# KUIS-AI-Tekalp-Research-Group/video-compression

Hardware: AMD Instinct MI355X
Metric: frames/sec + bpp/PSNR on UVG 1080p GOP-8, 1/2/4/8 MI355X (higher is better)
Workload: dtype f32; 1 GPU; LHBDC 1080p GOP-8 inference, single lambda: 7 B-frames per GOP via Model.forward, 4 independent GOP(s) per GPU per step, hierarchy levels batched across them; gop=8, resolution=1920x1080, precision=fp32, parallelism=gop-shard x1, launch=hip-graph per GOP pass

## Files before the change

video-compression_amd/csrc/conv_split.h:

```cpp
#pragma once
#include "conv_dma.h"

typedef short bf16x8 __attribute__((ext_vector_type(8)));

template <int K> struct SplitUnits {
    static constexpr int TPU = 4;
    static constexpr int Q = (K / 2) * (K / 2);
    static constexpr int V = (K + 3) / 4;
    static constexpr int H = (K - 1 + 3) / 4;
    static constexpr int U = Q + V + H;
    static constexpr int type(int u) { return u < Q ? 0 : (u < Q + V ? 1 : 2); }
    static constexpr int ky0(int u) { return u < Q ? 2 * (u / (K / 2)) : (u < Q + V ? 4 * (u - Q) : K - 1); }
    static constexpr int kx0(int u) { return u < Q ? 2 * (u % (K / 2)) : (u < Q + V ? K - 1 : 4 * (u - Q - V)); }
    static constexpr int nvalid(int u)
    {
        return u < Q ? 4 : (u < Q + V ? (K - 4 * (u - Q) < 4 ? K - 4 * (u - Q) : 4) : (K - 1 - 4 * (u - Q - V) < 4 ? K - 1 - 4 * (u - Q - V) : 4));
    }
    static constexpr int ky(int u, int q)
    {
        const int qq = q < nvalid(u) ? q : nvalid(u) - 1;
        return type(u) == 0 ? ky0(u) + (qq >> 1) : (type(u) == 1 ? ky0(u) + qq : ky0(u));
    }
    static constexpr int kx(int u, int q)
    {
// ... 158 lines not shown
#pragma unroll
        for (int nn = 0; nn < NG; ++nn) {
            const int n = n0 + nn;
            const int co = cur.nblk * C::BN + 16 * n + 4 * q;
            unsigned char *rec = sc + ((2 * nn + (q >> 1)) * 16 + px) * 48 + 8 * (q & 1);
            f32x4 v = acc[t][n];
            f32x4 r = {0.f, 0.f, 0.f, 0.f};
            if (p.res_sp3) {
                r = vc_load_split4(rec - 8 * (q & 1), q & 1);
            } else if (p.res) {
                if (pix_ok) r = *reinterpret_cast<const f32x4 *>(p.res + (long long)cur.img * p.res_sn + (long long)oy * p.res_sh + (long long)ox * p.res_sw + co);
            }
            if (p.res_first) v += r;
#pragma unroll
            for (int e = 0; e < 4; ++e) v[e] = v[e] >= 0.0f ? v[e] : v[e] * neg;
            if (p.chscale) v *= *reinterpret_cast<const f32x4 *>(p.chscale + co);
            if (p.res && !p.res_first) v += r;
            unsigned h[4], mm[4], l[4];
#pragma unroll
            for (int e = 0; e < 4; ++e) vc_split3(v[e], h[e], mm[e], l[e]);
            const u32x2 ph = {(h[0] >> 16) | h[1], (h[2] >> 16) | h[3]};
            const u32x2 pm = {(mm[0] >> 16) | mm[1], (mm[2] >> 16) | mm[3]};
            const u32x2 pl = {(l[0] >> 16) | (l[1] & 0xffff0000u), (l[2] >> 16) | (l[3] & 0xffff0000u)};
            if constexpr (C::KO & 256) {
                VC_DMA_KEEP(ph); VC_DMA_KEEP(pm); VC_DMA_KEEP(pl);
            } else {
                *reinterpret_cast<u32x2 *>(rec) = ph;
                *reinterpret_cast<u32x2 *>(rec + 16) = pm;
                *reinterpret_cast<u32x2 *>(rec + 32) = pl;
            }
        }
        if constexpr (C::KO & 256) continue;
        asm volatile("s_waitcnt lgkmcnt(0)" ::: "memory");
        const int plane0 = (cur.nblk * C::BN + 16 * n0) >> 3;
#pragma unroll
        for (int j = 0; j < NJ; ++j) {
            const bool ok = (64 * j + lane < UNITS) && row_ok && (oxb + u_w16[j] / 3 < p.Wo);
            if (ok) {
                const vc_u32x4 val = *reinterpret_cast<const vc_u32x4 *>(sc + u_plane[j] * 768 + u_w16[j] * 16);
                if constexpr (C::KO & 128) VC_DMA_KEEP(val);
                else *reinterpret_cast<vc_u32x4 *>(outb + ((((long long)(plane0 + u_plane[j])) * p.Ho + oy) * p.Wo + oxb) * 48 + u_w16[j] * 16) = val;
            }
        }
        asm volatile("s_waitcnt lgkmcnt(0)" ::: "memory");
    }
}

template <class C, int T0 = 0, int T1 = C::WM, int SC_NG = 0>
__device__ __forceinline__ void split_epilogue(const ConvArgs &p, f32x4 (&acc)[C::WM][C::WN], const DmaTile &cur, int wave, int px, int q,
                                               unsigned char *sc = nullptr)
{
    constexpr int WM = C::WM, WN = C::WN;
    if constexpr (SC_NG > 0 || (C::A_BYTES / 8 >= 3072 && WN % 2 == 0)) {
        if (sc && p.out_sp3 && p.out_mode == VC_OUT_PLAIN) {
            constexpr int NG = SC_NG > 0 ? SC_NG : ((C::A_BYTES / 8 >= WN * 1536) ? WN : 2);
            split_epilogue_records<C, NG, T0, T1>(p, acc, cur, wave, px, q, sc);
            return;
        }
    }
    const float neg = (p.act == VC_ACT_NONE) ? 1.0f : (p.act == VC_ACT_RELU ? 0.0f : p.slope);
#pragma unroll
    for (int t = T0; t < T1; ++t) {
        const int m = WM * wave + t;
        const int oy = cur.oy0 + (m >> 1), ox = cur.ox0 + 16 * (m & 1) + px;
        const bool pix_ok = oy < p.Ho && ox < p.Wo;
#pragma unroll
        for (int n = 0; n < WN; ++n) {
            const int co = cur.nblk * C::BN + 16 * n + 4 * q;
            const bool ok = pix_ok && co < p.Cout;
            f32x4 v = acc[t][n];
            f32x4 r = {0.f, 0.f, 0.f, 0.f};
            const bool ps = p.out_mode != VC_OUT_PLAIN;
            const int cps = p.Cout >> 2;
            const int pos = ps ? co / cps : 0;
            const int cch = ps ? co - pos * cps : co;
            const int yy = ps ? 2 * oy + (pos >> 1) : oy, xx = ps ? 2 * ox + (pos & 1) : ox;
            const int oh = ps ? 2 * p.Ho : p.Ho, ow = ps ? 2 * p.Wo : p.Wo;
            if (p.res_sp3) {
                if (ok) r = vc_load_split4(reinterpret_cast<const unsigned char *>(p.res) + (long long)cur.img * p.res_sn +
                                               ((((long long)(cch >> 3)) * oh + yy) * ow + xx) * 48, (cch >> 2) & 1);
            } else if (p.res) {
                const long long r_off = (long long)cur.img * p.res_sn + (long long)yy * p.res_sh + (long long)xx * p.res_sw + cch;
                if (ok) r = *reinterpret_cast<const f32x4 *>(p.res + r_off);
            }
            if (p.res_first) v += r;
#pragma unroll
            for (int e = 0; e < 4; ++e) v[e] = v[e] >= 0.0f ? v[e] : v[e] * neg;
            if (p.chscale) v *= *reinterpret_cast<const f32x4 *>(p.chscale + min(co, p.Cout - 4));
            if (p.res && !p.res_first) v += r;
            if (p.out_sp3) {
                unsigned char *o8 = reinterpret_cast<unsigned char *>(p.out) + (long long)cur.img * p.out_sn + ((((long long)(cch >> 3)) * oh + yy) * ow + xx) * 48;
                if (ok) vc_store_split4(o8, (cch >> 2) & 1, v);
            } else {
                const long long o_off = (long long)cur.img * p.out_sn + (long long)yy * p.out_sh + (long long)xx * p.out_sw + cch;
                if (ok) *reinterpret_cast<f32x4 *>(p.out + o_off) = v;
            }
        }
    }
}

template <class C> __global__ void __launch_bounds__(512, 2) conv_split_kernel(const ConvArgs p)
{
    typedef typename C::UN UN;
    constexpr int U = C::U, WM = C::WM, WN = C::WN, NA = C::NA, RING = C::RING, D = C::D, CPL = C::CPL;
    extern __shared__ __attribute__((aligned(16))) unsigned char lds8[];

    const int tid = threadIdx.x;
    const int lane = tid & 63;
    const int wave = __builtin_amdgcn_readfirstlane(tid >> 6);
    const int grp = wave >> 2;
    const int px = lane & 15, q = lane >> 4;

    const int per_img = p.tiles_x * p.tiles_y;
    const int total = per_img * p.N * p.nblks;
    const int xcd = blockIdx.x & 7, xl = blockIdx.x >> 3;
    const int tq = total >> 3, tr = total & 7;
    const int x_start = xcd * tq + min(xcd, tr), x_count = tq + (xcd < tr ? 1 : 0);
    auto tile_at = [&](int it) {
        DmaTile t;
        const int k = it * 32 + xl;
        t.valid = k < x_count;
        const int idx = x_start + (t.valid ? k : 0);
        t.nblk = idx % p.nblks;
        const int t1 = idx / p.nblks;
        t.img = t1 / per_img;
        int tx, ty;
        vc_tile_xy(t1 - t.img * per_img, p.tiles_x, p.tiles_y, p.tile_band, tx, ty);
        t.oy0 = ty * C::TH;
        t.ox0 = tx * C::TW;
        return t;
    };
    DmaTile cur = tile_at(0);
    if (!cur.valid) return;

    const int nchunk = p.Cin / (8 * CPL);
    const int upt = nchunk * U;
    const unsigned char *const in_b = reinterpret_cast<const unsigned char *>(p.in);
    const unsigned char *const wpk = reinterpret_cast<const unsigned char *>(p.wpk);
    const long long plane = (long long)p.H * p.W * C::PXB;
    const unsigned char *const zero_lane = g_vc_dma_zero + 16 * lane;

    int a_off[NA], a_rc[NA];
#pragma unroll
    for (int k = 0; k < NA; ++k) {
        const int s = k * 512 + tid;
        const int pl = s / C::PLANE_SLOTS, s2 = s - pl * C::PLANE_SLOTS;
        const int pix = s2 / 3, piece = s2 - 3 * pix;
        const int row = pix / C::COLS, col = pix - row * C::COLS;
        a_off[k] = pl * (int)plane + (row * p.W + col) * C::PXB + piece * 16;
        a_rc[k] = (pl < CPL && s2 < 3 * C::PIX) ? (row | (col << 8)) : 0x7f7f7f;
    }
    auto tile_base = [&](const DmaTile &t) {
        return in_b + (long long)t.img * p.in_sn + ((long long)(t.oy0 - C::PAD) * p.W + (t.ox0 - C::PAD)) * C::PXB;
    };
    auto issue_a = [&](const DmaTile &t, const unsigned char *tbase, int c, int k, int buf) {
        int rc = a_rc[k], off = a_off[k];
        asm volatile("" : "+v"(rc), "+v"(off));
        const unsigned iy = (unsigned)(t.oy0 - C::PAD + (rc & 0xff)), ix = (unsigned)(t.ox0 - C::PAD + (rc >> 8));
        const bool ok = t.valid && iy < (unsigned)p.H && ix < (unsigned)p.W;
        const unsigned char *sp = ok ? tbase + ((long long)c * CPL * plane + off) : zero_lane;
        if constexpr (!(C::KO & 16)) vc_glds16<true>(sp, (unsigned)(buf * C::A_BYTES + k * 8192 + wave * 1024));
    };
    const unsigned lane16 = 16 * lane;
    unsigned gbase = 0;
    auto issue_b = [&](int g, int nblk_cur, int nblk_next) {
        const int gg = g >= upt ? g - upt : g;
        const int nblk = g >= upt ? nblk_next : nblk_cur;
        const unsigned char *sbase = wpk + ((long long)nblk * upt + gg) * (C::FRAGS * 1024) + wave * 1024;
        const unsigned dst = C::B_OFF + ((gbase + (unsigned)g) % RING) * C::SLOTB + wave * 1024;
#pragma unroll
        for (int r = 0; r < C::ROUNDS; ++r)
            if constexpr (!(C::KO & 16)) {
                if (r + 1 < C::ROUNDS || !C::EXACT || grp == 0) vc_glds16_sbase(sbase + r * 8192, lane16, dst + r * 8192);
            }
    };

    float *const ldsf = reinterpret_cast<float *>(lds8);
    for (int i = tid; i < p.nblks * C::BN; i += 512) ldsf[C::BIAS_OFF / 4 + i] = p.bias[i];
    DmaTile nxt = tile_at(1);
    const unsigned char *cur_base = tile_base(cur), *nxt_base = tile_base(nxt);
#pragma unroll
    for (int k = 0; k < NA; ++k) issue_a(cur, cur_base, 0, k, 0);
#pragma unroll
    for (int g = 0; g < D; ++g) issue_b(g, cur.nblk, cur.nblk);
    vc_wait_vmcnt<0>();
    __syncthreads();

    constexpr bool TIMM = (WM % 2 == 0);
    const int qtap = q / CPL, qpl = q % CPL;
    int a_lane[UN::NCLS][TIMM ? 1 : WM];
#pragma unroll
    for (int c = 0; c < UN::NCLS; ++c) {
        int dy = 0, dx = 0;
#pragma unroll
        for (int qq = 0; qq < UN::TPU; ++qq)
            if (qtap == qq) {
                dy = UN::dy(c, qq);
                dx = UN::dx(c, qq);
            }
#pragma unroll
        for (int t = 0; t < (TIMM ? 1 : WM); ++t) {
            const int m = WM * wave + t;
            a_lane[c][t] = (((m >> 1) + dy) * C::COLS + 16 * (m & 1) + px + dx) * C::PXB + qpl * C::PLANE_B;
        }
    }
    const int b_lane = C::B_OFF + lane * 16;

    f32x4 acc[WM][WN];
    f32x4 af[3][WM], bf[3][WN];
    int gchunk = 0;
    for (int it = 0;; ++it) {
#pragma unroll
        for (int n = 0; n < WN; ++n) {
            const f32x4 b = *reinterpret_cast<const f32x4 *>(&ldsf[C::BIAS_OFF / 4 + cur.nblk * C::BN + 16 * n + 4 * q]);
#pragma unroll
            for (int t = 0; t < WM; ++t) acc[t][n] = b;
        }
        if (grp == 1) VC_DMA_BARRIER();
#pragma unroll 1
        for (int c = 0; c < nchunk; ++c) {
            const int abuf = ((gchunk + c) & 1) * C::A_BYTES, nbuf = ((gchunk + c + 1) & 1);
            const bool last_chunk = c + 1 == nchunk;
            const int g0 = c * U;
            static_for<0, U>([&](auto uc) {
                constexpr int u = decltype(uc)::value;
                constexpr int cl = UN::cls(u);
                const int bslot = b_lane + (int)((gbase + (unsigned)(g0 + u)) % RING) * C::SLOTB;
#pragma unroll
                for (int pc = 0; pc < 3; ++pc) {
#pragma unroll
                    for (int n = 0; n < WN; ++n) bf[pc][n] = *reinterpret_cast<const f32x4 *>(lds8 + bslot + (pc * WN + n) * 1024);
#pragma unroll
                    for (int t = 0; t < WM; ++t) {
                        const int ab = a_lane[cl][TIMM ? 0 : t] + abuf;
                        constexpr int unit_imm = (UN::ky0(u) * C::COLS + UN::kx0(u)) * C::PXB;
                        const int t_imm = TIMM ? ((t >> 1) * C::COLS + 16 * (t & 1)) * C::PXB : 0;
                        af[pc][t] = *reinterpret_cast<const f32x4 *>(lds8 + ab + unit_imm + t_imm + 16 * pc);
                    }
                }
                static_for<0, NA>([&](auto kc) {
                    constexpr int k = decltype(kc)::value;
                    if constexpr (C::piece_phase(k) == u) {
                        if (!last_chunk) issue_a(cur, cur_base, c + 1, k, nbuf);
                        else issue_a(nxt, nxt_base, 0, k, nbuf);
                    }
                });
                issue_b(g0 + u + D, cur.nblk, nxt.nblk);
                if constexpr (!(C::KO & 2)) {
                    if constexpr (C::nwait(u, 0) == C::nwait(u, 1)) vc_wait_vmcnt<C::nwait(u, 0)>();
                    else if (grp == 0) vc_wait_vmcnt<C::nwait(u, 0)>();
                    else vc_wait_vmcnt<C::nwait(u, 1)>();
                }
                VC_DMA_BARRIER();
                if constexpr (!(C::KO & 4)) {
                    __builtin_amdgcn_s_setprio(1);
#pragma unroll
                    for (int sum = 4; sum >= 0; --sum)
#pragma unroll
                        for (int pa = 2; pa >= 0; --pa) {
                            const int pb = sum - pa;
                            if (pb < 0 || pb > 2) continue;
#pragma unroll
                            for (int t = 0; t < WM; ++t)
#pragma unroll
                                for (int n = 0; n < WN; ++n)
                                    acc[t][n] = __builtin_amdgcn_mfma_f32_16x16x32_bf16(__builtin_bit_cast(bf16x8, bf[pb][n]),
                                                                                        __builtin_bit_cast(bf16x8, af[pa][t]), acc[t][n], 0, 0, 0);
                        }
                    __builtin_amdgcn_s_setprio(0);
                } else {
#pragma unroll
                    for (int pc = 0; pc < 3; ++pc) {
#pragma unroll
                        for (int t = 0; t < WM; ++t) VC_DMA_KEEP(af[pc][t]);
#pragma unroll
                        for (int n = 0; n < WN; ++n) VC_DMA_KEEP(bf[pc][n]);
                    }
                }
                VC_DMA_BARRIER();
            });
        }
        if (grp == 0) VC_DMA_BARRIER();
        gchunk += nchunk;
        gbase = (gbase + (unsigned)upt) % RING;

        if constexpr (!(C::KO & 1)) {
            split_epilogue<C>(p, acc, cur, wave, px, q);
        } else {
#pragma unroll
            for (int t = 0; t < WM; ++t)
#pragma unroll
                for (int n = 0; n < WN; ++n) VC_DMA_KEEP(acc[t][n]);
        }
        if (!nxt.valid) break;
        cur = nxt;
        cur_base = nxt_base;
        nxt = tile_at(it + 2);
        nxt_base = tile_base(nxt);
    }
    vc_wait_vmcnt<0>();
}

template <int K_, int NTW_, int TH_ = (K_ == 3 ? 12 : 16), int RING_ = 4, int KO_ = 0> struct SplitPeriodCfg {
    static constexpr int K = K_, NTW = NTW_, CPL = K_ == 3 ? 2 : 1, RING = RING_, KO = KO_, PAD = K_ / 2;
    static constexpr int KG = K_ * K_ * CPL, U = (2 * KG + 3) / 4;
    static constexpr int TH = TH_, TW = 32, BN = 16 * NTW_;
    static constexpr int WAVES = 8, WM = TH_ * 2 / 8, WN = NTW_;
    static_assert(WM * 8 == TH_ * 2, "the tile's 2 TH M-tiles split evenly over 8 waves");
    static constexpr int ROWS_IN = TH + K_ - 1, COLS = TW + K_ - 1, PIX = ROWS_IN * COLS, PXB = 48;
    static constexpr int PLANE_SLOTS = CPL == 1 ? 3 * PIX : (3 * PIX + 15) / 16 * 16, PLANE_B = PLANE_SLOTS * 16;
    static constexpr int NA = (CPL * PLANE_SLOTS + 511) / 512, A_BYTES = NA * 8192;
    static constexpr int FRAGS = 3 * NTW_, ROUNDS = (FRAGS + 7) / 8, LASTW = FRAGS - 8 * (ROUNDS - 1);
    static constexpr bool EXACT = LASTW == 4;
    static constexpr int SLOTB = EXACT ? FRAGS * 1024 : ROUNDS * 8192;
    static constexpr int nb(int grp) { return ROUNDS - ((EXACT && grp == 1) ? 1 : 0); }
    static constexpr int B_OFF = 2 * A_BYTES, BIAS_OFF = B_OFF + RING_ * SLOTB, LDS_FIXED = BIAS_OFF;
    static constexpr int D = RING_ - 2;
    static_assert(D == 2, "the issue windows below are laid out for weights requested two units ahead");
    static constexpr bool kg_valid(int u, int q) { return 4 * u + q < 2 * KG; }
    static constexpr int kg_chunk(int u, int q) { return kg_valid(u, q) ? (4 * u + q) / KG : 1; }
    static constexpr int kg_tap(int u, int q) { return kg_valid(u, q) ? ((4 * u + q) % KG) / CPL : 0; }
    static constexpr int kg_plane(int u, int q) { return kg_valid(u, q) ? ((4 * u + q) % KG) % CPL : 0; }
    static constexpr int XLAST = (KG - 1) / 4, YFIRST = KG / 4;
    static constexpr int YWIN = YFIRST - D, XWIN = U - D - XLAST - 1;
    static_assert(YWIN >= 1 && XWIN >= 1, "no issue window for a chunk image");
    static constexpr int PPP = (NA + (YWIN < XWIN ? YWIN : XWIN) - 1) / (YWIN < XWIN ? YWIN : XWIN);
    static constexpr int piece_phase(int which, int k) { return (which ? 1 : XLAST + 2) + k / PPP; }
    static_assert(piece_phase(1, NA - 1) <= YFIRST - D && piece_phase(0, NA - 1) <= U - D, "chunk image pieces outside their window");
    static constexpr int nA(int u)
    {
        int n = 0;
        for (int w = 0; w < 2; ++w)
            for (int k = 0; k < NA; ++k) n += piece_phase(w, k) == u;
        return n;
    }
    static constexpr int nwait(int u, int grp)
    {
        int n = 0;
        for (int j = u + 2 - D; j <= u; ++j) n += nA(((j % U) + U) % U) + nb(grp);
        return n;
    }
    static constexpr int max_wait()
    {
        int m = 0;
        for (int u = 0; u < U; ++u) m = nwait(u, 0) > m ? nwait(u, 0) : m;
        return m;
    }
    static_assert(max_wait() <= 63, "vmcnt is a 6-bit counter");
};

template <class C> __global__ void __launch_bounds__(512, 2) conv_split_period_kernel(const ConvArgs p)
{
    constexpr int U = C::U, WM = C::WM, WN = C::WN, NA = C::NA, RING = C::RING, D = C::D;
    extern __shared__ __attribute__((aligned(16))) unsigned char lds8[];
    const int tid = threadIdx.x;
    const int lane = tid & 63;
    const int wave = __builtin_amdgcn_readfirstlane(tid >> 6);
    const int grp = wave >> 2;
    const int px = lane & 15, q = lane >> 4;

    const int per_img = p.tiles_x * p.tiles_y;
    const int total = per_img * p.N * p.nblks;
    const int xcd = blockIdx.x & 7, xl = blockIdx.x >> 3;
    const int tq = total >> 3, tr = total & 7;
    const int x_start = xcd * tq + min(xcd, tr), x_count = tq + (xcd < tr ? 1 : 0);
    auto tile_at = [&](int it) {
        DmaTile t;
        const int k = it * 32 + xl;
        t.valid = k < x_count;
        const int idx = x_start + (t.valid ? k : 0);
        t.nblk = idx % p.nblks;
        const int t1 = idx / p.nblks;
        t.img = t1 / per_img;
        int tx, ty;
        vc_tile_xy(t1 - t.img * per_img, p.tiles_x, p.tiles_y, p.tile_band, tx, ty);
        t.oy0 = ty * C::TH;
        t.ox0 = tx * C::TW;
        return t;
    };
    DmaTile cur = tile_at(0);
    if (!cur.valid) return;

    const int nper = p.Cin / (16 * C::CPL);
    const int upt = nper * U;
    const unsigned char *const in_b = reinterpret_cast<const unsigned char *>(p.in);
    const unsigned char *const wpk = reinterpret_cast<const unsigned char *>(p.wpk);
    const long long plane = (long long)p.H * p.W * C::PXB;
    const unsigned char *const zero_lane = g_vc_dma_zero + 16 * lane;

    int a_off[NA], a_rc[NA];
#pragma unroll
    for (int k = 0; k < NA; ++k) {
        const int s = k * 512 + tid;
        const int pl = s / C::PLANE_SLOTS, s2 = s - pl * C::PLANE_SLOTS;
        const int pix = s2 / 3, piece = s2 - 3 * pix;
        const int row = pix / C::COLS, col = pix - row * C::COLS;
        a_off[k] = pl * (int)plane + (row * p.W + col) * C::PXB + piece * 16;
        a_rc[k] = (pl < C::CPL && s2 < 3 * C::PIX) ? (row | (col << 8)) : 0x7f7f7f;
    }
    auto tile_base = [&](const DmaTile &t) {
        return in_b + (long long)t.img * p.in_sn + ((long long)(t.oy0 - C::PAD) * p.W + (t.ox0 - C::PAD)) * C::PXB;
    };
    auto issue_a = [&](const DmaTile &t, const unsigned char *tbase, int c, int k, int buf) {
        int rc = a_rc[k], off = a_off[k];
        asm volatile("" : "+v"(rc), "+v"(off));
        const unsigned iy = (unsigned)(t.oy0 - C::PAD + (rc & 0xff)), ix = (unsigned)(t.ox0 - C::PAD + (rc >> 8));
        const bool ok = t.valid && iy < (unsigned)p.H && ix < (unsigned)p.W;
        const unsigned char *sp = ok ? tbase + ((long long)c * C::CPL * plane + off) : zero_lane;
        if constexpr (!(C::KO & 16)) vc_glds16<true>(sp, (unsigned)(buf * C::A_BYTES + k * 8192 + wave * 1024));
    };
    const unsigned lane16 = 16 * lane;
    unsigned gbase = 0;
    auto issue_b = [&](int g, int nblk_cur, int nblk_next) {
        const int gg = g >= upt ? g - upt : g;
        const int nblk = g >= upt ? nblk_next : nblk_cur;
        const unsigned char *sbase = wpk + ((long long)nblk * upt + gg) * (C::FRAGS * 1024) + wave * 1024;
        const unsigned dst = C::B_OFF + ((gbase + (unsigned)g) % RING) * C::SLOTB + wave * 1024;
#pragma unroll
        for (int r = 0; r < C::ROUNDS; ++r)
            if constexpr (!(C::KO & 16)) {
                if (r + 1 < C::ROUNDS || !C::EXACT || grp == 0) vc_glds16_sbase(sbase + r * 8192, lane16, dst + r * 8192);
            }
    };

    float *const ldsf = reinterpret_cast<float *>(lds8);
    for (int i = tid; i < p.nblks * C::BN; i += 512) ldsf[C::BIAS_OFF / 4 + i] = p.bias[i];
    DmaTile nxt = tile_at(1);
    const unsigned char *cur_base = tile_base(cur), *nxt_base = tile_base(nxt);
#pragma unroll
    for (int k = 0; k < NA; ++k) issue_a(cur, cur_base, 0, k, 0);
#pragma unroll
    for (int g = 0; g < D; ++g) issue_b(g, cur.nblk, cur.nblk);
    vc_wait_vmcnt<0>();
    __syncthreads();

    int a_t[WM], a_unit[U];
#pragma unroll
    for (int t = 0; t < WM; ++t) {
        const int m = WM * wave + t;
        a_t[t] = ((m >> 1) * C::COLS + 16 * (m & 1) + px) * C::PXB;
    }
#pragma unroll
    for (int u = 0; u < U; ++u) {
        int off = 0;
#pragma unroll
        for (int qq = 0; qq < 4; ++qq)
            if (q == qq)
                off = C::kg_chunk(u, qq) * C::A_BYTES + C::kg_plane(u, qq) * C::PLANE_B + ((C::kg_tap(u, qq) / C::K) * C::COLS + C::kg_tap(u, qq) % C::K) * C::PXB;
        a_unit[u] = off;
    }
    const int b_lane = C::B_OFF + lane * 16;

#ifdef VC_DMA_DIAG
    unsigned st_sum[8] = {0, 0, 0, 0, 0, 0, 0, 0};
#endif
    VC_DMA_STAMP(t_begin);
    f32x4 acc[WM][WN];
    f32x4 af[3][WM], bf[3][WN];
    for (int it = 0;; ++it) {
#pragma unroll
        for (int n = 0; n < WN; ++n) {
            const f32x4 b = *reinterpret_cast<const f32x4 *>(&ldsf[C::BIAS_OFF / 4 + cur.nblk * C::BN + 16 * n + 4 * q]);
#pragma unroll
            for (int t = 0; t < WM; ++t) acc[t][n] = b;
        }
        if (grp == 1) VC_DMA_BARRIER();
#pragma unroll 1
        for (int pr = 0; pr < nper; ++pr) {
            const bool last_per = pr + 1 == nper;
            const int g0 = pr * U;
            static_for<0, U>([&](auto uc) {
                constexpr int u = decltype(uc)::value;
                VC_DMA_STAMP(t0);
                const int bslot = b_lane + (int)((gbase + (unsigned)(g0 + u)) % RING) * C::SLOTB;
#pragma unroll
                for (int pc = 0; pc < 3; ++pc) {
#pragma unroll
                    for (int n = 0; n < WN; ++n) bf[pc][n] = *reinterpret_cast<const f32x4 *>(lds8 + bslot + (pc * WN + n) * 1024);
#pragma unroll
                    for (int t = 0; t < WM; ++t) af[pc][t] = *reinterpret_cast<const f32x4 *>(lds8 + (a_t[t] + a_unit[u]) + 16 * pc);
                }
                VC_DMA_STAMP(t1);
                static_for<0, NA>([&](auto kc) {
                    constexpr int k = decltype(kc)::value;
                    if constexpr (C::piece_phase(1, k) == u) issue_a(cur, cur_base, 2 * pr + 1, k, 1);
                    if constexpr (C::piece_phase(0, k) == u) {
                        if (!last_per) issue_a(cur, cur_base, 2 * pr + 2, k, 0);
                        else issue_a(nxt, nxt_base, 0, k, 0);
                    }
                });
                issue_b(g0 + u + D, cur.nblk, nxt.nblk);
                VC_DMA_STAMP(t2);
                if constexpr (!(C::KO & 2)) {
                    if constexpr (C::nwait(u, 0) == C::nwait(u, 1)) vc_wait_vmcnt<C::nwait(u, 0)>();
                    else if (grp == 0) vc_wait_vmcnt<C::nwait(u, 0)>();
                    else vc_wait_vmcnt<C::nwait(u, 1)>();
                }
                VC_DMA_STAMP(t3);
                VC_DMA_BARRIER();
                VC_DMA_STAMP(t4);
                if constexpr (!(C::KO & 4)) {
                    __builtin_amdgcn_s_setprio(1);
#pragma unroll
                    for (int sum = 4; sum >= 0; --sum)
#pragma unroll
                        for (int pa = 2; pa >= 0; --pa) {
                            const int pb = sum - pa;
                            if (pb < 0 || pb > 2) continue;
#pragma unroll
                            for (int t = 0; t < WM; ++t)
#pragma unroll
                                for (int n = 0; n < WN; ++n)
                                    acc[t][n] = __builtin_amdgcn_mfma_f32_16x16x32_bf16(__builtin_bit_cast(bf16x8, bf[pb][n]),
                                                                                        __builtin_bit_cast(bf16x8, af[pa][t]), acc[t][n], 0, 0, 0);
                        }
                    __builtin_amdgcn_s_setprio(0);
                } else {
#pragma unroll
                    for (int pc = 0; pc < 3; ++pc) {
#pragma unroll
                        for (int t = 0; t < WM; ++t) VC_DMA_KEEP(af[pc][t]);
#pragma unroll
                        for (int n = 0; n < WN; ++n) VC_DMA_KEEP(bf[pc][n]);
                    }
                }
                VC_DMA_STAMP(t5);
                VC_DMA_BARRIER();
                VC_DMA_STAMP(t6);
                VC_DMA_ACC(0, t2, t1);
                VC_DMA_ACC(1, t1, t0);
                VC_DMA_ACC(2, t3, t2);
                VC_DMA_ACC(3, t4, t3);
                VC_DMA_ACC(4, t5, t4);
                VC_DMA_ACC(5, t6, t5);
            });
        }
        if (grp == 0) VC_DMA_BARRIER();
        gbase = (gbase + (unsigned)upt) % RING;
        VC_DMA_STAMP(t_e0);
        if constexpr (!(C::KO & 1)) {
            split_epilogue<C>(p, acc, cur, wave, px, q, (C::KO & 32) ? nullptr : lds8 + C::A_BYTES + wave * (C::A_BYTES / 8));
        } else {
#pragma unroll
            for (int t = 0; t < WM; ++t)
#pragma unroll
                for (int n = 0; n < WN; ++n) VC_DMA_KEEP(acc[t][n]);
        }
        VC_DMA_STAMP(t_e1);
        VC_DMA_ACC(6, t_e1, t_e0);
        if (!nxt.valid) break;
        cur = nxt;
        cur_base = nxt_base;
        nxt = tile_at(it + 2);
        nxt_base = tile_base(nxt);
    }
    vc_wait_vmcnt<0>();
#ifdef VC_DMA_DIAG
    if constexpr (C::KO & 64) {
        VC_DMA_STAMP(t_end);
        st_sum[7] = t_end - t_begin;
        if (lane == 0)
            for (int i = 0; i < 8; ++i) atomicAdd(&g_vc_dma_stamps[i], (unsigned long long)st_sum[i]);
    }
#endif
}

template <class C> int launch_conv_split_period(hipStream_t st, const ConvArgs &a)
{
    const size_t lds_bytes = C::LDS_FIXED + (size_t)a.nblks * C::BN * sizeof(float);
    if (lds_bytes > 160 * 1024) return VC_EINVAL;
    auto kern = conv_split_period_kernel<C>;
    static vc_lds_raised raised;
    if (!vc_raise_lds_limit(reinterpret_cast<const void *>(kern), lds_bytes, raised)) return VC_ELAUNCH;
    hipLaunchKernelGGL(kern, dim3(256), dim3(512), lds_bytes, st, a);
    return hipGetLastError() == hipSuccess ? VC_OK : VC_ELAUNCH;
}

template <class C> int launch_conv_split(hipStream_t st, const ConvArgs &a)
{
    const size_t lds_bytes = C::LDS_FIXED + (size_t)a.nblks * C::BN * sizeof(float);
    if (lds_bytes > 160 * 1024) return VC_EINVAL;
    auto kern = conv_split_kernel<C>;
    static vc_lds_raised raised;
    if (!vc_raise_lds_limit(reinterpret_cast<const void *>(kern), lds_bytes, raised)) return VC_ELAUNCH;
    hipLaunchKernelGGL(kern, dim3(256), dim3(512), lds_bytes, st, a);
    return hipGetLastError() == hipSuccess ? VC_OK : VC_ELAUNCH;
}
```

video-compression_amd/csrc/conv_split.hip:

```cpp
#include <stdlib.h>
#include <string.h>
#include "conv_split.h"

static inline unsigned short bf16_trunc_bits(float x)
{
    unsigned u;
    memcpy(&u, &x, 4);
    return (unsigned short)(u >> 16);
}
static inline float bf16_bits_to_float(unsigned short h)
{
    const unsigned u = (unsigned)h << 16;
    float f;
    memcpy(&f, &u, 4);
    return f;
}
static inline void split3_host(float x, unsigned short pc[3])
{
    pc[0] = bf16_trunc_bits(x);
    const float r1 = x - bf16_bits_to_float(pc[0]);
    pc[1] = bf16_trunc_bits(r1);
    const float r2 = r1 - bf16_bits_to_float(pc[1]);
    pc[2] = bf16_trunc_bits(r2);
}

static int split_cpl(int k) { return k == 3 ? 2 : ((k == 5 || k == 7) ? 1 : 0); }
static int split_units(int k)
{
    return k == 7 ? SplitUnits<7>::U : (k == 5 ? SplitUnits<5>::U : (k == 3 ? SplitPairs<3>::U : 0));
}
static int split_block(int cout, int k)
{
    if (k == 3) return (cout % 64 == 0) ? 64 : ((cout % 32 == 0) ? 32 : 0);
    return (cout % 64 == 0) ? 64 : ((cout % 32 == 0) ? 32 : ((k == 7 && cout % 16 == 0) ? 16 : 0));
}

extern "C" size_t vc_conv_packed_weight_bytes_split(int cout, int cin, int k)
{
    const int u = split_units(k), bn = split_block(cout, k), cpl = split_cpl(k);
    if (!u || !bn || !cpl || (cin % (8 * cpl))) return 0;
    return (size_t)(cout / bn) * (cin / (8 * cpl)) * u * 3 * (bn / 16) * 1024 + 16384;
}

template <class UN, int K, int CPL> static void pack_split(const float *w, int cout, int cin, int bn, int ps, unsigned short *dst)
{
    const int ntw = bn / 16, nchunk = cin / (8 * CPL), cps = cout / 4;
    for (int nb = 0; nb < cout / bn; ++nb)
        for (int c = 0; c < nchunk; ++c)
            for (int u = 0; u < UN::U; ++u) {
                unsigned short *unit = dst + (((size_t)nb * nchunk + c) * UN::U + u) * (3 * ntw * 512);
                for (int n = 0; n < ntw; ++n)
                    for (int lane = 0; lane < 64; ++lane) {
                        const int cop = nb * bn + 16 * n + (lane & 15), q = lane >> 4;
                        const int co = ps ? (cop % cps) * 4 + cop / cps : cop;
                        const int tap = q / CPL, pl = q % CPL;
                        for (int j = 0; j < 8; ++j) {
                            unsigned short pc[3] = {0, 0, 0};
                            if (UN::valid(u, tap))
                                split3_host(w[(((size_t)co * cin + (c * CPL + pl) * 8 + j) * K + UN::ky(u, tap)) * K + UN::kx(u, tap)], pc);
                            for (int piece = 0; piece < 3; ++piece) unit[((piece * ntw + n) * 64 + lane) * 8 + j] = pc[piece];
                        }
                    }
            }
}

template <int K> static void pack_split_period(const float *w, int cout, int cin, int bn, int ps, unsigned short *dst)
{
    typedef SplitPeriodCfg<K, 4> C;
    constexpr int CPL = C::CPL, KG = C::KG, U = C::U;
    const int ntw = bn / 16, nper = cin / (16 * CPL), cps = cout / 4;
    for (int nb = 0; nb < cout / bn; ++nb)
        for (int pr = 0; pr < nper; ++pr)
            for (int u = 0; u < U; ++u) {
                unsigned short *unit = dst + (((size_t)nb * nper + pr) * U + u) * (3 * ntw * 512);
                for (int n = 0; n < ntw; ++n)
                    for (int lane = 0; lane < 64; ++lane) {
                        const int cop = nb * bn + 16 * n + (lane & 15), q = lane >> 4;
                        const int co = ps ? (cop % cps) * 4 + cop / cps : cop;
                        const int g = 4 * u + q;
                        if (g >= 2 * KG) continue;
                        const int chunk = g / KG, tap = (g % KG) / CPL, pl = (g % KG) % CPL;
                        for (int j = 0; j < 8; ++j) {
                            unsigned short pc[3];
                            split3_host(w[(((size_t)co * cin + (2 * pr + chunk) * 8 * CPL + 8 * pl + j) * K + tap / K) * K + tap % K], pc);
                            for (int piece = 0; piece < 3; ++piece) unit[((piece * ntw + n) * 64 + lane) * 8 + j] = pc[piece];
                        }
                    }
            }
}
static bool split_period(int k, int cin, int bn)
{
    if (bn == 16) return false;
    static const bool padded = [] {
        const char *e = getenv("VC_SPLIT_PADDED"), *e3 = getenv("VC_SPLIT3_PADDED");
        return (e && e[0] && e[0] != '0') || (e3 && e3[0] && e3[0] != '0');
    }();
    if (padded) return false;
    return (k == 3 && (cin % 32) == 0) || ((k == 5 || k == 7) && (cin % 16) == 0);
}

extern "C" int vc_conv_pack_weights_split(const float *w, const float *bias, int cout, int cin, int k, int pixelshuffle, void *wpk_out,
                                          float *bias_out)
{
    const size_t bytes = vc_conv_packed_weight_bytes_split(cout, cin, k);
    if (!w || !wpk_out || !bias_out || !bytes || (pixelshuffle && (cout % 16))) return VC_EINVAL;
    memset(wpk_out, 0, bytes);
    unsigned short *dst = static_cast<unsigned short *>(wpk_out);
    const int bn = split_block(cout, k);
    if (split_period(k, cin, bn)) {
        if (k == 7) pack_split_period<7>(w, cout, cin, bn, pixelshuffle, dst);
        else if (k == 5) pack_split_period<5>(w, cout, cin, bn, pixelshuffle, dst);
        else pack_split_period<3>(w, cout, cin, bn, pixelshuffle, dst);
    } else if (k == 7) pack_split<SplitUnits<7>, 7, 1>(w, cout, cin, bn, pixelshuffle, dst);
    else if (k == 5) pack_split<SplitUnits<5>, 5, 1>(w, cout, cin, bn, pixelshuffle, dst);
    else pack_split<SplitPairs<3>, 3, 2>(w, cout, cin, bn, pixelshuffle, dst);
    const int cps = cout / 4;
    for (int cop = 0; cop < cout; ++cop) {
        const int co = pixelshuffle ? (cop % cps) * 4 + cop / cps : cop;
        bias_out[cop] = bias ? bias[co] : 0.0f;
    }
    return VC_OK;
}

template <int PB> __global__ void __launch_bounds__(256) k_split3(vc_view a, unsigned char *__restrict__ out, long long out_img_bytes)
{
    __shared__ __attribute__((aligned(16))) unsigned char sm[VC_RECORDS_LDS(PB)];
    const int nb = (a.c >> 3) / PB;
    const int x_run = (int)blockIdx.x * (256 / PB);
    const int gi = threadIdx.x % PB, x = x_run + (int)threadIdx.x / PB, y = blockIdx.y;
    const int n = blockIdx.z / nb, g0 = (blockIdx.z - n * nb) * PB;
    vc_u32x4 ph = {0, 0, 0, 0}, pm = ph, pl = ph;
    if (x < a.w) {
        const float *src = a.p + view_off(a, n, y, x) + 8 * (g0 + gi);
        vc_split_record(*reinterpret_cast<const f32x4 *>(src), *reinterpret_cast<const f32x4 *>(src + 4), ph, pm, pl);
    }
    const long long plane_bytes = (long long)a.h * a.w * 48;
    vc_store_records_256<PB>(sm, threadIdx.x, x < a.w, ph, pm, pl, out + n * out_img_bytes + g0 * plane_bytes + ((long long)y * a.w + x_run) * 48,
                             plane_bytes, min(256 / PB, a.w - x_run));
}

extern "C" int vc_split3(vc_stream s, vc_view a, void *out_split, long long out_image_bytes)
{
    if (!a.p || !out_split || (a.c % 8) || (a.sw % 4) || (a.sh % 4) || (a.sn % 4) || ((uintptr_t)a.p % 16) || ((uintptr_t)out_split % 16) ||
        (out_image_bytes % 16))
        return VC_EINVAL;
    const long long total = (long long)a.n * (a.c / 8) * a.h * a.w;
    if (total <= 0) return VC_OK;
    const long long img = out_image_bytes ? out_image_bytes : (long long)(a.c / 8) * a.h * a.w * 48;
    unsigned char *o = static_cast<unsigned char *>(out_split);
    const int cg = a.c / 8;
    const int pb = cg % 8 == 0 ? 8 : (cg % 4 == 0 ? 4 : (cg % 2 == 0 ? 2 : 1));
    const long long gz = (long long)a.n * (cg / pb);
    if (a.h > 65535 || gz > 65535) return VC_EINVAL;
    const dim3 grid((unsigned)((a.w + 256 / pb - 1) / (256 / pb)), (unsigned)a.h, (unsigned)gz);
    if (pb == 8) hipLaunchKernelGGL(k_split3<8>, grid, dim3(256), 0, as_stream(s), a, o, img);
    else if (pb == 4) hipLaunchKernelGGL(k_split3<4>, grid, dim3(256), 0, as_stream(s), a, o, img);
    else if (pb == 2) hipLaunchKernelGGL(k_split3<2>, grid, dim3(256), 0, as_stream(s), a, o, img);
    else hipLaunchKernelGGL(k_split3<1>, grid, dim3(256), 0, as_stream(s), a, o, img);
    VC_LAUNCH_CHECK();
    return VC_OK;
}

int conv_dispatch_split(hipStream_t st, ConvArgs a, int k, int stride)
{
    const int cpl = split_cpl(k);
    if (stride != 1 || !cpl || !a.in_sp3 || a.in_f16 || a.out_f16 || a.res_f16 || a.tail_wpk || a.epi != VC_EPI_NONE || a.in_xform != VC_IN_NONE ||
        (a.Cin % (8 * cpl)) || a.act == VC_ACT_SIGMOID || a.act == VC_ACT_CLAMP01)
        return VC_EINVAL;
    const int bn = split_block(a.Cout, k);
    if (!bn) return VC_EINVAL;
    const int cpp = a.out_mode == VC_OUT_PLAIN ? a.Cout : a.Cout / 4;
    if (a.out_mode != VC_OUT_PLAIN && (a.Cout % 16)) return VC_EINVAL;
    if (a.out_sp3 ? (cpp % 8 != 0) : !a.vec_out) return VC_EINVAL;
    if ((long long)cpl * a.H * a.W * 48 + (long long)(k + 15) * a.W * 48 + 48ll * 48 >= (1ll << 31)) return VC_EINVAL;
    if (a.res_sp3 && (!a.res || (cpp % 8))) return VC_EINVAL;
    if (!a.in_sn) a.in_sn = (long long)(a.Cin / 8) * a.H * a.W * 48;
    const int osc = a.out_mode == VC_OUT_PLAIN ? 1 : 2;
    if (a.out_sp3 && !a.out_sn) a.out_sn = (long long)(cpp / 8) * osc * a.Ho * osc * a.Wo * 48;
    if (a.res_sp3 && !a.res_sn) a.res_sn = (long long)(cpp / 8) * osc * a.Ho * osc * a.Wo * 48;
    if ((a.in_sn % 16) || (a.out_sp3 && (a.out_sn % 16)) || (a.res_sp3 && (a.res_sn % 8))) return VC_EINVAL;
    const int th = k == 3 ? 12 : (bn == 16 ? 24 : 16);
    a.tiles_x = (a.Wo + 31) / 32;
    a.tiles_y = (a.Ho + th - 1) / th;
    a.nblks = a.Cout / bn;
    a.total_blocks = a.tiles_x * a.tiles_y * a.nblks * a.N;
#ifdef VC_SPLIT_DIAG
    {
        const char *e = getenv("VC_SPLIT_VARIANT");
        const int v = e ? atoi(e) : 0;
#ifdef VC_DMA_DIAG
        if (k == 3 && split_period(k, a.Cin, bn) && bn == 64) {
            if (v == 64 + 128) return launch_conv_split_period<SplitPeriodCfg<3, 4, 12, 4, 64 + 128>>(st, a);
            if (v == 64 + 256) return launch_conv_split_period<SplitPeriodCfg<3, 4, 12, 4, 64 + 256>>(st, a);
            if (v == 64 + 32) return launch_conv_split_period<SplitPeriodCfg<3, 4, 12, 4, 64 + 32>>(st, a);
        }
        if (v == 64 && split_period(k, a.Cin, bn) && bn == 64) {
            if (k == 3) return launch_conv_split_period<SplitPeriodCfg<3, 4, 12, 4, 64>>(st, a);
            if (k == 7) return launch_conv_split_period<SplitPeriodCfg<7, 4, 16, 4, 64>>(st, a);
        }
#endif
        if (k == 7 && bn == 64) {
            switch (v) {
            case 1: return launch_conv_split<SplitCfg<7, 4, 1, 16, 4, 1>>(st, a);
            case 4: return launch_conv_split<SplitCfg<7, 4, 1, 16, 4, 4>>(st, a);
            case 16: return launch_conv_split<SplitCfg<7, 4, 1, 16, 4, 16>>(st, a);
            case 17: return launch_conv_split<SplitCfg<7, 4, 1, 16, 4, 17>>(st, a);
            case 21: return launch_conv_split<SplitCfg<7, 4, 1, 16, 4, 21>>(st, a);
            }
        }
    }
#endif
    if (split_period(k, a.Cin, bn)) {
        if (k == 7) return bn == 64 ? launch_conv_split_period<SplitPeriodCfg<7, 4>>(st, a) : launch_conv_split_period<SplitPeriodCfg<7, 2>>(st, a);
        if (k == 5) return bn == 64 ? launch_conv_split_period<SplitPeriodCfg<5, 4>>(st, a) : launch_conv_split_period<SplitPeriodCfg<5, 2>>(st, a);
        return bn == 64 ? launch_conv_split_period<SplitPeriodCfg<3, 4>>(st, a) : launch_conv_split_period<SplitPeriodCfg<3, 2>>(st, a);
    }
    if (k == 7 && bn == 16) return launch_conv_split<SplitCfg<7, 1, 1, 24>>(st, a);
    if (k == 7) return bn == 64 ? launch_conv_split<SplitCfg<7, 4>>(st, a) : launch_conv_split<SplitCfg<7, 2>>(st, a);
    if (k == 5) return bn == 64 ? launch_conv_split<SplitCfg<5, 4>>(st, a) : launch_conv_split<SplitCfg<5, 2>>(st, a);
    if (k == 3) return bn == 64 ? launch_conv_split<SplitCfg<3, 4, 2, 12>>(st, a) : launch_conv_split<SplitCfg<3, 2, 2, 12>>(st, a);
    return VC_EINVAL;
}

#if defined(VC_SPLIT_DIAG) && defined(VC_DMA_DIAG)
extern "C" int vc_debug_dma_stamps(unsigned long long *out8)
{
    if (hipDeviceSynchronize() != hipSuccess) return VC_ELAUNCH;
    if (hipMemcpyFromSymbol(out8, HIP_SYMBOL(g_vc_dma_stamps), 8 * sizeof(unsigned long long)) != hipSuccess) return VC_ELAUNCH;
    unsigned long long zero[8] = {0};
    if (hipMemcpyToSymbol(HIP_SYMBOL(g_vc_dma_stamps), zero, sizeof(zero)) != hipSuccess) return VC_ELAUNCH;
    return VC_OK;
}
#endif
```

Before: 22.24 frames/s.

## Use 16-row tiles with a rotating triple input buffer for 3x3 split convs

For 3x3 convolutions with 64-wide output blocks, the period kernel now uses 16-row tiles and one input plane per chunk. Four chunks are processed per period, rotating through three LDS input image buffers, and the chunk-prefetch issue windows are generalised to N chunks over M buffers. The aim is to amortise the halo rows and weight traffic over more output rows per tile. In exchange it uses more LDS (three A buffers), which may reduce occupancy, and adds buffer-rotation arithmetic. An environment variable falls back to the 12-row path.

Result: no change. 22.32 frames/s, median of 6 (+0.4%).

```diff
diff --git a/video-compression_amd/csrc/conv_split.h b/video-compression_amd/csrc/conv_split.h
--- a/video-compression_amd/csrc/conv_split.h
+++ b/video-compression_amd/csrc/conv_split.h
@@ -484,8 +484,10 @@
 }
 
 template <int K_, int NTW_, int TH_ = (K_ == 3 ? 12 : 16), int RING_ = 4, int KO_ = 0> struct SplitPeriodCfg {
-    static constexpr int K = K_, NTW = NTW_, CPL = K_ == 3 ? 2 : 1, RING = RING_, KO = KO_, PAD = K_ / 2;
-    static constexpr int KG = K_ * K_ * CPL, U = (2 * KG + 3) / 4;
+    static constexpr bool ROT = K_ == 3 && TH_ == 16;
+    static constexpr int K = K_, NTW = NTW_, CPL = (K_ == 3 && !ROT) ? 2 : 1, RING = RING_, KO = KO_, PAD = K_ / 2;
+    static constexpr int NCH = ROT ? 4 : 2, NBUF = ROT ? 3 : 2;
+    static constexpr int KG = K_ * K_ * CPL, U = (NCH * KG + 3) / 4;
     static constexpr int TH = TH_, TW = 32, BN = 16 * NTW_;
     static constexpr int WAVES = 8, WM = TH_ * 2 / 8, WN = NTW_;
     static_assert(WM * 8 == TH_ * 2, "the tile's 2 TH M-tiles split evenly over 8 waves");
@@ -496,24 +498,42 @@
     static constexpr bool EXACT = LASTW == 4;
     static constexpr int SLOTB = EXACT ? FRAGS * 1024 : ROUNDS * 8192;
     static constexpr int nb(int grp) { return ROUNDS - ((EXACT && grp == 1) ? 1 : 0); }
-    static constexpr int B_OFF = 2 * A_BYTES, BIAS_OFF = B_OFF + RING_ * SLOTB, LDS_FIXED = BIAS_OFF;
+    static constexpr int B_OFF = NBUF * A_BYTES, BIAS_OFF = B_OFF + RING_ * SLOTB, LDS_FIXED = BIAS_OFF;
     static constexpr int D = RING_ - 2;
     static_assert(D == 2, "the issue windows below are laid out for weights requested two units ahead");
-    static constexpr bool kg_valid(int u, int q) { return 4 * u + q < 2 * KG; }
-    static constexpr int kg_chunk(int u, int q) { return kg_valid(u, q) ? (4 * u + q) / KG : 1; }
+    static constexpr bool kg_valid(int u, int q) { return 4 * u + q < NCH * KG; }
+    static constexpr int kg_chunk(int u, int q) { return kg_valid(u, q) ? (4 * u + q) / KG : NCH - 1; }
     static constexpr int kg_tap(int u, int q) { return kg_valid(u, q) ? ((4 * u + q) % KG) / CPL : 0; }
     static constexpr int kg_plane(int u, int q) { return kg_valid(u, q) ? ((4 * u + q) % KG) % CPL : 0; }
-    static constexpr int XLAST = (KG - 1) / 4, YFIRST = KG / 4;
-    static constexpr int YWIN = YFIRST - D, XWIN = U - D - XLAST - 1;
-    static_assert(YWIN >= 1 && XWIN >= 1, "no issue window for a chunk image");
-    static constexpr int PPP = (NA + (YWIN < XWIN ? YWIN : XWIN) - 1) / (YWIN < XWIN ? YWIN : XWIN);
-    static constexpr int piece_phase(int which, int k) { return (which ? 1 : XLAST + 2) + k / PPP; }
-    static_assert(piece_phase(1, NA - 1) <= YFIRST - D && piece_phase(0, NA - 1) <= U - D, "chunk image pieces outside their window");
+    static constexpr int fdiv(int a, int b) { return (a >= 0 ? a : a - b + 1) / b; }
+    static constexpr int first(int a) { return fdiv(a, NCH) * U + ((a - fdiv(a, NCH) * NCH) * KG) / 4; }
+    static constexpr int last(int a) { return fdiv(a, NCH) * U + ((a - fdiv(a, NCH) * NCH) * KG + KG - 1) / 4; }
+    static constexpr int win_lo(int c) { return last(c - NBUF) + 2; }
+    static constexpr int win_hi(int c) { return first(c) - D; }
+    static constexpr int win_min()
+    {
+        int m = U;
+        for (int c = 0; c < NCH; ++c) m = win_hi(c) - win_lo(c) + 1 < m ? win_hi(c) - win_lo(c) + 1 : m;
+        return m;
+    }
+    static_assert(win_min() >= 1, "no issue window for a chunk image");
+    static constexpr int ppp(int c) { return ROT ? (NA + win_hi(c) - win_lo(c)) / (win_hi(c) - win_lo(c) + 1) : (NA + win_min() - 1) / win_min(); }
+    static constexpr int fill_t(int c, int k) { return win_lo(c) + k / ppp(c); }
+    static constexpr bool fill_next(int c, int k) { return fill_t(c, k) < 0; }
+    static constexpr int fill_phase(int c, int k) { return fill_t(c, k) < 0 ? fill_t(c, k) + U : fill_t(c, k); }
+    static constexpr bool fills_ok()
+    {
+        for (int c = 0; c < NCH; ++c)
+            for (int k = 0; k < NA; ++k)
+                if (fill_t(c, k) > win_hi(c) || fill_t(c, k) < -U || fill_phase(c, k) >= U) return false;
+        return true;
+    }
+    static_assert(fills_ok(), "chunk image pieces outside their window");
     static constexpr int nA(int u)
     {
         int n = 0;
-        for (int w = 0; w < 2; ++w)
-            for (int k = 0; k < NA; ++k) n += piece_phase(w, k) == u;
+        for (int c = 0; c < NCH; ++c)
+            for (int k = 0; k < NA; ++k) n += fill_phase(c, k) == u;
         return n;
     }
     static constexpr int nwait(int u, int grp)
@@ -530,10 +550,19 @@
     }
     static_assert(max_wait() <= 63, "vmcnt is a 6-bit counter");
 };
+static_assert(SplitPeriodCfg<7, 4>::fill_phase(1, 0) == 1 && !SplitPeriodCfg<7, 4>::fill_next(1, 0) && SplitPeriodCfg<7, 4>::fill_phase(0, 0) == 14 &&
+              SplitPeriodCfg<7, 4>::fill_next(0, 0) && SplitPeriodCfg<3, 4>::fill_phase(0, 0) == 6 && SplitPeriodCfg<3, 4>::fill_phase(0, 5) == 7 &&
+              SplitPeriodCfg<3, 4>::fill_phase(1, 5) == 2, "two-chunk periods: the issue phases of rounds 5 and 6");
+static_assert(SplitPeriodCfg<3, 4, 16>::NA == 4 && SplitPeriodCfg<3, 4, 16>::U == 9 && SplitPeriodCfg<3, 4, 16>::fill_phase(2, 0) == 1 &&
+              SplitPeriodCfg<3, 4, 16>::fill_phase(2, 3) == 2 && SplitPeriodCfg<3, 4, 16>::fill_phase(3, 0) == 4 && SplitPeriodCfg<3, 4, 16>::fill_phase(3, 3) == 4 &&
+              SplitPeriodCfg<3, 4, 16>::fill_phase(0, 0) == 6 && SplitPeriodCfg<3, 4, 16>::fill_next(0, 3) && SplitPeriodCfg<3, 4, 16>::fill_phase(0, 3) == 7 &&
+              SplitPeriodCfg<3, 4, 16>::fill_phase(1, 1) == 8 && SplitPeriodCfg<3, 4, 16>::fill_next(1, 1) && SplitPeriodCfg<3, 4, 16>::fill_phase(1, 2) == 0 &&
+              !SplitPeriodCfg<3, 4, 16>::fill_next(1, 2), "16-row 3 x 3 instance: the issue phases");
 
 template <class C> __global__ void __launch_bounds__(512, 2) conv_split_period_kernel(const ConvArgs p)
 {
-    constexpr int U = C::U, WM = C::WM, WN = C::WN, NA = C::NA, RING = C::RING, D = C::D;
+    constexpr int U = C::U, WM = C::WM, WN = C::WN, NA = C::NA, RING = C::RING, D = C::D, NCH = C::NCH, NBUF = C::NBUF;
+    constexpr bool ROT = NCH % NBUF != 0;
     extern __shared__ __attribute__((aligned(16))) unsigned char lds8[];
     const int tid = threadIdx.x;
     const int lane = tid & 63;
@@ -563,7 +592,7 @@
     DmaTile cur = tile_at(0);
     if (!cur.valid) return;
 
-    const int nper = p.Cin / (16 * C::CPL);
+    const int nper = p.Cin / (8 * C::CPL * NCH);
     const int upt = nper * U;
     const unsigned char *const in_b = reinterpret_cast<const unsigned char *>(p.in);
     const unsigned char *const wpk = reinterpret_cast<const unsigned char *>(p.wpk);
@@ -609,8 +638,12 @@
     for (int i = tid; i < p.nblks * C::BN; i += 512) ldsf[C::BIAS_OFF / 4 + i] = p.bias[i];
     DmaTile nxt = tile_at(1);
     const unsigned char *cur_base = tile_base(cur), *nxt_base = tile_base(nxt);
-#pragma unroll
-    for (int k = 0; k < NA; ++k) issue_a(cur, cur_base, 0, k, 0);
+    static_for<0, NCH>([&](auto cc) {
+        static_for<0, NA>([&](auto kc) {
+            constexpr int c = decltype(cc)::value, k = decltype(kc)::value;
+            if constexpr (C::fill_next(c, k)) issue_a(cur, cur_base, c, k, c % NBUF);
+        });
+    });
 #pragma unroll
     for (int g = 0; g < D; ++g) issue_b(g, cur.nblk, cur.nblk);
     vc_wait_vmcnt<0>();
@@ -639,6 +672,7 @@
     VC_DMA_STAMP(t_begin);
     f32x4 acc[WM][WN];
     f32x4 af[3][WM], bf[3][WN];
+    int bsel = 0;
     for (int it = 0;; ++it) {
 #pragma unroll
         for (int n = 0; n < WN; ++n) {
@@ -655,21 +689,29 @@
                 constexpr int u = decltype(uc)::value;
                 VC_DMA_STAMP(t0);
                 const int bslot = b_lane + (int)((gbase + (unsigned)(g0 + u)) % RING) * C::SLOTB;
+                int a_u = a_unit[u];
+                if constexpr (ROT) {
+                    a_u += bsel * C::A_BYTES;
+                    a_u = (int)min((unsigned)a_u, (unsigned)a_u - (unsigned)(NBUF * C::A_BYTES));
+                }
 #pragma unroll
                 for (int pc = 0; pc < 3; ++pc) {
 #pragma unroll
                     for (int n = 0; n < WN; ++n) bf[pc][n] = *reinterpret_cast<const f32x4 *>(lds8 + bslot + (pc * WN + n) * 1024);
 #pragma unroll
-                    for (int t = 0; t < WM; ++t) af[pc][t] = *reinterpret_cast<const f32x4 *>(lds8 + (a_t[t] + a_unit[u]) + 16 * pc);
+                    for (int t = 0; t < WM; ++t) af[pc][t] = *reinterpret_cast<const f32x4 *>(lds8 + (a_t[t] + a_u) + 16 * pc);
                 }
                 VC_DMA_STAMP(t1);
                 static_for<0, NA>([&](auto kc) {
-                    constexpr int k = decltype(kc)::value;
-                    if constexpr (C::piece_phase(1, k) == u) issue_a(cur, cur_base, 2 * pr + 1, k, 1);
-                    if constexpr (C::piece_phase(0, k) == u) {
-                        if (!last_per) issue_a(cur, cur_base, 2 * pr + 2, k, 0);
-                        else issue_a(nxt, nxt_base, 0, k, 0);
-                    }
+                    static_for<0, NCH>([&](auto cc) {
+                        constexpr int k = decltype(kc)::value, c = NCH - 1 - decltype(cc)::value;
+                        if constexpr (C::fill_phase(c, k) == u) {
+                            constexpr int ahead = C::fill_next(c, k) ? NCH : 0;
+                            const int buf = ROT ? (bsel + ahead + c) % NBUF : c;
+                            if (!ahead || !last_per) issue_a(cur, cur_base, NCH * pr + ahead + c, k, buf);
+                            else issue_a(nxt, nxt_base, c, k, buf);
+                        }
+                    });
                 });
                 issue_b(g0 + u + D, cur.nblk, nxt.nblk);
                 VC_DMA_STAMP(t2);
@@ -716,12 +758,14 @@
                 VC_DMA_ACC(4, t5, t4);
                 VC_DMA_ACC(5, t6, t5);
             });
+            if constexpr (ROT) bsel = (bsel + NCH) % NBUF;
         }
         if (grp == 0) VC_DMA_BARRIER();
         gbase = (gbase + (unsigned)upt) % RING;
         VC_DMA_STAMP(t_e0);
+        const int ebuf = ROT ? (bsel + NBUF - 1) % NBUF : 1;
         if constexpr (!(C::KO & 1)) {
-            split_epilogue<C>(p, acc, cur, wave, px, q, (C::KO & 32) ? nullptr : lds8 + C::A_BYTES + wave * (C::A_BYTES / 8));
+            split_epilogue<C>(p, acc, cur, wave, px, q, (C::KO & 32) ? nullptr : lds8 + ebuf * C::A_BYTES + wave * (C::A_BYTES / 8));
         } else {
 #pragma unroll
             for (int t = 0; t < WM; ++t)
diff --git a/video-compression_amd/csrc/conv_split.hip b/video-compression_amd/csrc/conv_split.hip
--- a/video-compression_amd/csrc/conv_split.hip
+++ b/video-compression_amd/csrc/conv_split.hip
@@ -64,11 +64,10 @@
             }
 }
 
-template <int K> static void pack_split_period(const float *w, int cout, int cin, int bn, int ps, unsigned short *dst)
-{
-    typedef SplitPeriodCfg<K, 4> C;
-    constexpr int CPL = C::CPL, KG = C::KG, U = C::U;
-    const int ntw = bn / 16, nper = cin / (16 * CPL), cps = cout / 4;
+template <class C> static void pack_split_period(const float *w, int cout, int cin, int bn, int ps, unsigned short *dst)
+{
+    constexpr int K = C::K, CPL = C::CPL, KG = C::KG, U = C::U, NCH = C::NCH;
+    const int ntw = bn / 16, nper = cin / (8 * CPL * NCH), cps = cout / 4;
     for (int nb = 0; nb < cout / bn; ++nb)
         for (int pr = 0; pr < nper; ++pr)
             for (int u = 0; u < U; ++u) {
@@ -78,11 +77,11 @@
                         const int cop = nb * bn + 16 * n + (lane & 15), q = lane >> 4;
                         const int co = ps ? (cop % cps) * 4 + cop / cps : cop;
                         const int g = 4 * u + q;
-                        if (g >= 2 * KG) continue;
+                        if (g >= NCH * KG) continue;
                         const int chunk = g / KG, tap = (g % KG) / CPL, pl = (g % KG) % CPL;
                         for (int j = 0; j < 8; ++j) {
                             unsigned short pc[3];
-                            split3_host(w[(((size_t)co * cin + (2 * pr + chunk) * 8 * CPL + 8 * pl + j) * K + tap / K) * K + tap % K], pc);
+                            split3_host(w[(((size_t)co * cin + (NCH * pr + chunk) * 8 * CPL + 8 * pl + j) * K + tap / K) * K + tap % K], pc);
                             for (int piece = 0; piece < 3; ++piece) unit[((piece * ntw + n) * 64 + lane) * 8 + j] = pc[piece];
                         }
                     }
@@ -98,6 +97,11 @@
     if (padded) return false;
     return (k == 3 && (cin % 32) == 0) || ((k == 5 || k == 7) && (cin % 16) == 0);
 }
+static bool split3_rows16(int k, int cin, int bn)
+{
+    static const bool rows12 = [] { const char *e = getenv("VC_SPLIT3_ROWS12"); return e && e[0] && e[0] != '0'; }();
+    return k == 3 && bn == 64 && !rows12 && split_period(k, cin, bn);
+}
 
 extern "C" int vc_conv_pack_weights_split(const float *w, const float *bias, int cout, int cin, int k, int pixelshuffle, void *wpk_out,
                                           float *bias_out)
@@ -108,9 +112,10 @@
     unsigned short *dst = static_cast<unsigned short *>(wpk_out);
     const int bn = split_block(cout, k);
     if (split_period(k, cin, bn)) {
-        if (k == 7) pack_split_period<7>(w, cout, cin, bn, pixelshuffle, dst);
-        else if (k == 5) pack_split_period<5>(w, cout, cin, bn, pixelshuffle, dst);
-        else pack_split_period<3>(w, cout, cin, bn, pixelshuffle, dst);
+        if (k == 7) pack_split_period<SplitPeriodCfg<7, 4>>(w, cout, cin, bn, pixelshuffle, dst);
+        else if (k == 5) pack_split_period<SplitPeriodCfg<5, 4>>(w, cout, cin, bn, pixelshuffle, dst);
+        else if (split3_rows16(k, cin, bn)) pack_split_period<SplitPeriodCfg<3, 4, 16>>(w, cout, cin, bn, pixelshuffle, dst);
+        else pack_split_period<SplitPeriodCfg<3, 4>>(w, cout, cin, bn, pixelshuffle, dst);
     } else if (k == 7) pack_split<SplitUnits<7>, 7, 1>(w, cout, cin, bn, pixelshuffle, dst);
     else if (k == 5) pack_split<SplitUnits<5>, 5, 1>(w, cout, cin, bn, pixelshuffle, dst);
     else pack_split<SplitPairs<3>, 3, 2>(w, cout, cin, bn, pixelshuffle, dst);
@@ -179,7 +184,8 @@
     if (a.out_sp3 && !a.out_sn) a.out_sn = (long long)(cpp / 8) * osc * a.Ho * osc * a.Wo * 48;
     if (a.res_sp3 && !a.res_sn) a.res_sn = (long long)(cpp / 8) * osc * a.Ho * osc * a.Wo * 48;
     if ((a.in_sn % 16) || (a.out_sp3 && (a.out_sn % 16)) || (a.res_sp3 && (a.res_sn % 8))) return VC_EINVAL;
-    const int th = k == 3 ? 12 : (bn == 16 ? 24 : 16);
+    const bool rows16 = split3_rows16(k, a.Cin, bn);
+    const int th = k == 3 ? (rows16 ? 16 : 12) : (bn == 16 ? 24 : 16);
     a.tiles_x = (a.Wo + 31) / 32;
     a.tiles_y = (a.Ho + th - 1) / th;
     a.nblks = a.Cout / bn;
@@ -190,15 +196,20 @@
         const int v = e ? atoi(e) : 0;
 #ifdef VC_DMA_DIAG
         if (k == 3 && split_period(k, a.Cin, bn) && bn == 64) {
-            if (v == 64 + 128) return launch_conv_split_period<SplitPeriodCfg<3, 4, 12, 4, 64 + 128>>(st, a);
-            if (v == 64 + 256) return launch_conv_split_period<SplitPeriodCfg<3, 4, 12, 4, 64 + 256>>(st, a);
-            if (v == 64 + 32) return launch_conv_split_period<SplitPeriodCfg<3, 4, 12, 4, 64 + 32>>(st, a);
+            if (v == 64 + 128) return rows16 ? launch_conv_split_period<SplitPeriodCfg<3, 4, 16, 4, 64 + 128>>(st, a)
+                                             : launch_conv_split_period<SplitPeriodCfg<3, 4, 12, 4, 64 + 128>>(st, a);
+            if (v == 64 + 256) return rows16 ? launch_conv_split_period<SplitPeriodCfg<3, 4, 16, 4, 64 + 256>>(st, a)
+                                             : launch_conv_split_period<SplitPeriodCfg<3, 4, 12, 4, 64 + 256>>(st, a);
+            if (v == 64 + 32) return rows16 ? launch_conv_split_period<SplitPeriodCfg<3, 4, 16, 4, 64 + 32>>(st, a)
+                                            : launch_conv_split_period<SplitPeriodCfg<3, 4, 12, 4, 64 + 32>>(st, a);
         }
         if (v == 64 && split_period(k, a.Cin, bn) && bn == 64) {
-            if (k == 3) return launch_conv_split_period<SplitPeriodCfg<3, 4, 12, 4, 64>>(st, a);
+            if (k == 3) return rows16 ? launch_conv_split_period<SplitPeriodCfg<3, 4, 16, 4, 64>>(st, a) : launch_conv_split_period<SplitPeriodCfg<3, 4, 12, 4, 64>>(st, a);
             if (k == 7) return launch_conv_split_period<SplitPeriodCfg<7, 4, 16, 4, 64>>(st, a);
         }
 #endif
+        if (v == 1 && k == 3 && split_period(k, a.Cin, bn) && bn == 64)
+            return rows16 ? launch_conv_split_period<SplitPeriodCfg<3, 4, 16, 4, 1>>(st, a) : launch_conv_split_period<SplitPeriodCfg<3, 4, 12, 4, 1>>(st, a);
         if (k == 7 && bn == 64) {
             switch (v) {
             case 1: return launch_conv_split<SplitCfg<7, 4, 1, 16, 4, 1>>(st, a);
@@ -213,6 +224,7 @@
     if (split_period(k, a.Cin, bn)) {
         if (k == 7) return bn == 64 ? launch_conv_split_period<SplitPeriodCfg<7, 4>>(st, a) : launch_conv_split_period<SplitPeriodCfg<7, 2>>(st, a);
         if (k == 5) return bn == 64 ? launch_conv_split_period<SplitPeriodCfg<5, 4>>(st, a) : launch_conv_split_period<SplitPeriodCfg<5, 2>>(st, a);
+        if (rows16) return launch_conv_split_period<SplitPeriodCfg<3, 4, 16>>(st, a);
         return bn == 64 ? launch_conv_split_period<SplitPeriodCfg<3, 4>>(st, a) : launch_conv_split_period<SplitPeriodCfg<3, 2>>(st, a);
     }
     if (k == 7 && bn == 16) return launch_conv_split<SplitCfg<7, 1, 1, 24>>(st, a);
```
